# xbarin02/libdwt

Measured on AMD Instinct MI355X. Metric: Gsamples/s (= % HBM3E BW) CDF 9/7 2-D fwd float, 8192^2 5-level, higher is better.
Workload: dtype f32

## Files before the change

libdwt_amd/csrc/dwt_abi.hip:

```cpp
#include "dwt_backend.h"

#include <climits>

using namespace dwtb;

namespace {
enum OptKind { kPlain, kSweep , kBool, kNonNegative, kRing01 ,
	kUpDown01  };
struct Opt {
	const char *name;
	int *(*ref)(Ctx &);
	OptKind kind;
};
#define DWT_OPT(name_, member_, kind_) {name_, [](Ctx &c) -> int * { return &c.member_; }, kind_}
const Opt kOpts[] = {
	DWT_OPT("generic", force_generic, kSweep), DWT_OPT("eaw_two_pass", eaw_two_pass, kBool), DWT_OPT("feat_groups", feat_groups, kNonNegative), DWT_OPT("swt_fused", swt_fused, kBool), DWT_OPT("swt2d_fused", swt2d_fused, kBool), DWT_OPT("wp_fused", wp_fused, kBool), DWT_OPT("pixels_wide", pixels_wide, kBool), DWT_OPT("quant_wide", quant_wide, kBool), DWT_OPT("sparse_wide", sparse_wide, kBool), DWT_OPT("window_fused", window_fused, kNonNegative), DWT_OPT("cond_fused", cond_fused, kPlain), DWT_OPT("timefreq_tiled", tf_tiled, kBool), DWT_OPT("cpt", tune.cpt, kSweep), DWT_OPT("tile_pairs", tune.tile_pairs, kSweep),
	DWT_OPT("waves", tune.waves, kSweep), DWT_OPT("xcd_swizzle", tune.xcd_swizzle, kSweep), DWT_OPT("ring", tune.ring, kSweep),
	DWT_OPT("ring_inv", tune.ring_inv, kSweep), DWT_OPT("inv_ll_temporal", tune.inv_ll_temporal, kSweep), DWT_OPT("inv_pairs", tune.inv_pairs, kSweep), DWT_OPT("nt", tune.nt, kSweep), DWT_OPT("nt_auto", tune.nt_auto, kSweep),
	DWT_OPT("fma", fma, kSweep), DWT_OPT("fused_d", fused_d, kPlain), DWT_OPT("fuse01", fuse01, kPlain), DWT_OPT("fuse01_ring", tune.fuse01_ring, kRing01), DWT_OPT("fuse01_updown", tune.fuse01_updown, kUpDown01), DWT_OPT("ride_copy", ride_copy, kBool), DWT_OPT("ride_mib", ride_mib, kNonNegative), DWT_OPT("il_exact_borders", il_exact_borders, kPlain),
	DWT_OPT("il_inplace_shell", il_inplace_shell, kPlain), DWT_OPT("host_pipeline", host_pipeline, kPlain),
	DWT_OPT("tune_tiles", tune_tiles, kPlain), DWT_OPT("tune_in_call", tune_in_call, kBool), DWT_OPT("place_tries", place_tries, kPlain),
	DWT_OPT("place_min_mib", place_min_mib, kNonNegative), DWT_OPT("place_max_gib", place_max_gib, kNonNegative),
	DWT_OPT("vol_ip_waves", vol.ip_waves, kPlain), DWT_OPT("vol_tile_pairs", vol.tile_pairs, kPlain), DWT_OPT("vol_nt", vol.nt, kPlain),
	DWT_OPT("vol_fused", vol.fused, kPlain), DWT_OPT("vol_direct", vol.direct, kPlain), DWT_OPT("vol_whole", vol.whole, kPlain),
	DWT_OPT("vol_inplace_fused", vol.inplace_fused, kBool), DWT_OPT("vol_swizzle", vol.swizzle, kPlain), DWT_OPT("vol_rows", vol.rows, kPlain),
};
#undef DWT_OPT
const Opt *find_opt(const char *name)
{
	for (const Opt &o : kOpts)
		if (!strcmp(name, o.name))
			return &o;
	return nullptr;
}
}

#pragma GCC visibility push(default)
extern "C" {

const char *dwt_hip_last_error(void) { return g_err; }

int dwt_hip_device_count(void)
{
	int n = 0;
	if (hipGetDeviceCount(&n) != hipSuccess)
		return 0;
	return n;
}

int dwt_hip_init(void)
{
	if (g.inited)
		return 0;
	int n = 0;
	hipError_t e = hipGetDeviceCount(&n);
	if (e != hipSuccess || n <= 0)
		return fail("no HIP device available (%s); libdwt_amd has no CPU fallback", e != hipSuccess ? hipGetErrorString(e) : "0 devices");
	int dev = 0;
	const char *env = getenv("DWT_HIP_DEVICE");
	if (!env)
		env = getenv("LOCAL_RANK");
	if (g.want_device >= 0) {
		if (g.want_device >= n)
			return fail("dwt_hip_set_device(%d): the process sees %d device(s)", g.want_device, n);
		dev = g.want_device;
	} else if (env) {
		dev = atoi(env) % n;
	}
	HIP_TRY(hipSetDevice(dev));
	hipDeviceProp_t prop;
	HIP_TRY(hipGetDeviceProperties(&prop, dev));
	snprintf(g.devname, sizeof(g.devname), "%s (%s, %d CUs)", prop.name, prop.gcnArchName, prop.multiProcessorCount);
	if (!strstr(prop.gcnArchName, "gfx950"))
		return fail("device %d is %s; this library carries gfx950 code only", dev, prop.gcnArchName);
	g.device = dev;
	g.inited = true;
	return 0;
}

int dwt_hip_set_device(int device)
{
	if (device < 0)
		return fail("dwt_hip_set_device(%d): bad device index", device);
	if (g.inited && g.device != device) {
		dwt_hip_finish();
		g.inited = false;
	}
	g.want_device = device;
	return check_inited();
}

int dwt_hip_get_device(void)
{
	return g.inited ? g.device : -1;
}

void dwt_hip_finish(void)
{
	if (!g.inited)
		return;
	hipStreamSynchronize(g.stream);
	if (g.ll_external) {
		g.ll[0] = g.ll[1] = Buf{};
		g.ll_external = false;
	}
	for (Buf *b : g.bufs())
		drop(*b);
	for (hipEvent_t &e : g.dl_ev) {
		if (e)
			hipEventDestroy(e);
		e = nullptr;
	}
	for (auto &row : g.pipe_ev)
		for (hipEvent_t &e : row) {
			if (e)
				hipEventDestroy(e);
			e = nullptr;
		}
	if (g.up)
		hipStreamDestroy(g.up);
	if (g.down)
		hipStreamDestroy(g.down);
	g.up = g.down = nullptr;
	if (g.pin)
		hipHostFree(g.pin);
	g.pin = nullptr;
	g.pin_bytes = 0;
	if (g.switch_ev)
		hipEventDestroy(g.switch_ev);
	g.switch_ev = nullptr;
	for (auto &ev : g.prof_events) {
		hipEventDestroy(ev.first);
		hipEventDestroy(ev.second);
	}
	g.prof_events.clear();
	g.prof_used = 0;
	g.tile_cache.clear();
	g.place_n = 0;
	g.place_best = -1;
}

const char *dwt_hip_device_name(void)
{
	if (check_inited())
		return "";
	return g.devname;
}

void dwt_hip_set_stream(void *s)
{
	hipStream_t ns = (hipStream_t)s;
	if (g.inited && ns != g.stream) {
		hipStreamCaptureStatus a = hipStreamCaptureStatusNone, b = hipStreamCaptureStatusNone;
		const bool plain = hipStreamIsCapturing(g.stream, &a) == hipSuccess && a == hipStreamCaptureStatusNone &&
			hipStreamIsCapturing(ns, &b) == hipSuccess && b == hipStreamCaptureStatusNone;
		if (plain && (g.switch_ev || hipEventCreateWithFlags(&g.switch_ev, hipEventDisableTiming) == hipSuccess) &&
			hipEventRecord(g.switch_ev, g.stream) == hipSuccess)
			(void)hipStreamWaitEvent(ns, g.switch_ev, 0);
		(void)hipGetLastError();
	}
	g.stream = ns;
}

int dwt_hip_set_workspace(void *band0, size_t bytes0, void *band1, size_t bytes1)
{
	if (check_inited())
		return 1;
	HIP_TRY(hipStreamSynchronize(g.stream));
	if (!g.ll_external) {
		drop(g.ll[0]);
		drop(g.ll[1]);
	}
	if (!band0 || !band1) {
		g.ll[0] = g.ll[1] = Buf{};
		g.ll_external = false;
		return 0;
	}
	if (!dwt_hip_is_device_pointer(band0) || !dwt_hip_is_device_pointer(band1) || ((uintptr_t)band0 & 15) || ((uintptr_t)band1 & 15))
		return fail("dwt_hip_set_workspace takes two 16-byte aligned device buffers");
	g.ll[0] = Buf{band0, bytes0};
	g.ll[1] = Buf{band1, bytes1};
	g.ll_external = true;
	return 0;
}

int dwt_hip_fill_workspace(unsigned word)
{
	if (check_inited())
		return 1;
	for (Buf *b : g.bufs()) {
		if (!b->p || !b->bytes)
			continue;
		const size_t words = b->bytes / 4;
		if (words)
			HIP_TRY(hipMemsetD32Async((hipDeviceptr_t)b->p, (int)word, words, g.stream));
		for (size_t k = 4 * words; k < b->bytes; k++)
			HIP_TRY(hipMemsetD8Async((hipDeviceptr_t)((char *)b->p + k), (unsigned char)(word >> (8 * (k & 3))), 1, g.stream));
	}
	cond_forget_warnings();
	return 0;
}

int dwt_hip_placement_report(double *ms, int n)
{
	for (int i = 0; i < n && i < g.place_n; i++)
		ms[i] = g.place_ms[i];
	return g.place_n;
}


void dwt_hip_sync(void)
{
	if (g.inited)
		hipStreamSynchronize(g.stream);
}

int dwt_hip_set_option(const char *name, int value)
{
	const Opt *o = name ? find_opt(name) : nullptr;
	if (!o)
		return fail("unknown option '%s'", name ? name : "(null)");
	if (o->kind == kRing01 && value != 0 && !fwd01_has_ring(value))
		return fail("option fuse01_ring: 0, 8 or 16 (the fused pair has no kernel with a ring of %d rows)", value);
	if (o->kind == kUpDown01 && !fwd01_has_updown(value))
		return fail("option fuse01_updown: -1 (the rule), 0, 1 or 2, not %d", value);
	if (o->kind == kSweep || o->kind == kRing01 || o->kind == kUpDown01)
		g.tile_cache.clear();
	*o->ref(g) = o->kind == kBool ? (value ? 1 : 0) : (o->kind == kNonNegative && value < 0) ? 0 : value;
	return 0;
}

int dwt_hip_get_option(const char *name)
{
	if (!name)
		return -1;
	if (!strcmp(name, "tune_in_call"))
		return may_measure() && !g.tuning ? 1 : 0;
	if (!strcmp(name, "place_last_tries"))
		return g.place_n;
	if (!strcmp(name, "place_last_best"))
		return g.place_best;
	if (!strcmp(name, "stat_launches"))
		return (int)(g.stat_launches & 0x7fffffff);
	if (!strcmp(name, "stat_allocs"))
		return (int)(g.stat_allocs & 0x7fffffff);
	if (!strcmp(name, "tile_cache_size"))
		return (int)g.tile_cache.size();
	if (!strcmp(name, "fuse01_last_choice"))
		return g.stat_choice01;
	if (!strcmp(name, "fuse01_last_updown"))
		return g.stat_updown01;
	const Opt *o = find_opt(name);
	return o ? *o->ref(g) : -1;
}

int dwt_hip_is_device_pointer(const void *p)
{
	hipPointerAttribute_t at;
	hipError_t e = hipPointerGetAttributes(&at, p);
	if (e != hipSuccess) {
		(void)hipGetLastError();
		return 0;
	}
	return at.type == hipMemoryTypeDevice || at.type == hipMemoryTypeManaged;
}

void *dwt_hip_malloc(size_t bytes)
{
	if (check_inited())
		return nullptr;
	void *p = nullptr;
	if (hipMalloc(&p, bytes) != hipSuccess) {
		fail("hipMalloc(%zu) failed", bytes);
		return nullptr;
	}
	return p;
}

void dwt_hip_free(void *p)
{
	dev_free(p);
}

void *dwt_hip_malloc_host(size_t bytes)
{
	if (check_inited())
		return nullptr;
	void *p = nullptr;
	if (hipHostMalloc(&p, bytes, hipHostMallocDefault) != hipSuccess) {
		fail("hipHostMalloc(%zu) failed", bytes);
		return nullptr;
	}
	return p;
}

void dwt_hip_free_host(void *p)
{
	if (p)
		hipHostFree(p);
}

int dwt_hip_memcpy_h2d(void *d, const void *h, size_t n)
{
	if (check_inited())
		return 1;
	HIP_TRY(hipMemcpyAsync(d, h, n, hipMemcpyHostToDevice, g.stream));
	HIP_TRY(hipStreamSynchronize(g.stream));
	return 0;
}

int dwt_hip_memcpy_d2h(void *h, const void *d, size_t n)
{
	if (check_inited())
		return 1;
	HIP_TRY(hipMemcpyAsync(h, d, n, hipMemcpyDeviceToHost, g.stream));
	HIP_TRY(hipStreamSynchronize(g.stream));
	return 0;
}

void dwt_hip_prof_enable(int on)
{
	if (g.inited)
		prof_drain();
	g.prof_on = on;
	g.prof_ms = 0;
	g.prof_launches = 0;
}

int dwt_hip_prof_read_levels(double *ms_sum, int *launches, int n)
{
	if (prof_drain())
		return 1;
	for (int i = 0; i < n && i < 16; i++) {
		ms_sum[i] = g.prof_level_ms[i];
		launches[i] = g.prof_level_n[i];
		g.prof_level_ms[i] = 0;
		g.prof_level_n[i] = 0;
	}
	g.prof_ms = 0;
	g.prof_launches = 0;
	return 0;
}

int dwt_hip_prof_read(double *ms, int *launches)
{
	if (prof_drain())
		return 1;
	if (ms)
		*ms = g.prof_ms;
	if (launches)
		*launches = g.prof_launches;
	g.prof_ms = 0;
	g.prof_launches = 0;
	for (int i = 0; i < 16; i++) {
		g.prof_level_ms[i] = 0;
		g.prof_level_n[i] = 0;
	}
	return 0;
}
int dwt_hip_transform2d(int wavelet, int inverse, const void *src, void *dst, int stride_x, int stride_y,
	int sox, int soy, int six, int siy, int *j, int decompose_one, int zero_padding)
{
	if (check_inited())
		return 1;
	Wavelet w;
	if (!wavelet_of(wavelet, &w))
		return fail("unknown wavelet %d", wavelet);
	if (!src || !dst || !j)
		return fail("null pointer argument");
	Call2d c = call2d(w, {src, dst}, {(long)stride_x});
	const int es = c.es;
	if (sox <= 0 || soy <= 0 || six < 0 || siy < 0 || six > sox || siy > soy)
		return fail("bad sizes: outer %dx%d inner %dx%d", sox, soy, six, siy);
	const Geom ge{sox, soy, six, siy};
	const bool dev_src = dwt_hip_is_device_pointer(src), dev_dst = dwt_hip_is_device_pointer(dst);
	if (dev_src != dev_dst)
		return fail("src and dst must both be host or both be device pointers");

	if (dev_dst && stride_y == es && stride_x % es == 0 && stride_x >= sox * es && (uintptr_t)src % es == 0 && (uintptr_t)dst % es == 0) {
		Img s{(char *)src, stride_x, es}, d{(char *)dst, stride_x, es};
		if (!inverse && !decompose_one && (*j < 0 || *j >= 2) && place_ll_scratch(c, s, d, ge, *j, 1, 0, 0))
			return 1;
		return inverse ? inverse2d(c, s, d, ge, *j, decompose_one, zero_padding, 1, 0, 0)
		               : forward2d(c, s, d, ge, j, decompose_one, zero_padding, 1, 0, 0);
	}
	if (dev_dst && (stride_y < es || (long)stride_x < (long)(sox - 1) * stride_y + es))
		return fail("device image: stride_y %d must be >= %d and stride_x %d >= (width-1)*stride_y + %d", stride_y, es, stride_x, es);

	if (!dev_dst && ge.dense() && stride_y == es && es == 4) {
		const int rc = inverse ? host_inverse_pipelined(c, src, dst, stride_x, sox, soy, *j, decompose_one)
		                       : host_forward_pipelined(c, src, dst, stride_x, sox, soy, j, decompose_one);
		if (rc >= 0)
			return rc;
	}
	const bool s2 = (src != dst);
	const Frame fs{(void *)src, stride_x, stride_y, es, sox, soy, dev_dst}, fd{dst, stride_x, stride_y, es, sox, soy, dev_dst};
	Img A;
	if (frame_stage(fs, g.frame_a, &A) || grow(g.frame_b, (size_t)A.sx * soy))
		return 1;
	const long pitch = A.sx;
	const Img B{(char *)g.frame_b.p, pitch, es};
	c = call2d(w, {A.p, B.p}, {pitch});
	const int so_min = sox < soy ? sox : soy, so_max = sox > soy ? sox : soy;
	const int j_lim = ceil_log2(decompose_one ? so_max : so_min);
	const int j_eff = (*j < 0 || *j > j_lim) ? j_lim : *j;
	const bool writes_all = ge.dense() && j_eff >= 1;
	if (s2 && writes_all) {
	} else if (s2) {
		if (frame_pack(fd, B.p, pitch))
			return 1;
	} else {
		if (copy_rect(B, 0, 0, A, 0, 0, sox, soy))
			return 1;
	}
	int rc;
	if (s2 || ge.dense()) {
		rc = inverse ? inverse2d(c, A, B, ge, *j, decompose_one, zero_padding, 1, 0, 0)
		             : forward2d(c, A, B, ge, j, decompose_one, zero_padding, 1, 0, 0);
	} else {
		rc = inverse ? inverse2d(c, B, B, ge, *j, decompose_one, zero_padding, 1, 0, 0)
		             : forward2d(c, B, B, ge, j, decompose_one, zero_padding, 1, 0, 0);
	}
	if (rc)
		return rc;
	return frame_unpack(fd, B.p, pitch);
}

int dwt_hip_transform1d_batch(int wavelet, int inverse, const void *src, void *dst, size_t line_stride, int elem_stride,
	int n_lines, int size_o, int size_i, int *j, int zero_padding)
{
	if (check_inited())
		return 1;
	if (wavelet != DWT_HIP_CDF97_S && wavelet != DWT_HIP_CDF53_S && wavelet != DWT_HIP_INTERP53_S)
		return fail("1-D transforms exist for DWT_HIP_CDF97_S, DWT_HIP_CDF53_S and DWT_HIP_INTERP53_S only (wavelet %d)", wavelet);
	Wavelet w;
	wavelet_of(wavelet, &w);
	if (!src || !dst || !j)
		return fail("null pointer argument");
	if (n_lines < 0 || size_o < 0 || size_i < 0 || size_i > size_o)
		return fail("bad sizes: %d lines, outer %d inner %d", n_lines, size_o, size_i);
	if (elem_stride < 4 || line_stride > (size_t)LONG_MAX / 2)
		return fail("bad strides: line %zu bytes, element %d bytes", line_stride, elem_stride);
	return transform1d(w, inverse != 0, src, dst, (long)line_stride, elem_stride, n_lines, size_o, size_i, j, zero_padding);
}

int dwt_hip_transform1d(int wavelet, int inverse, const void *src, void *dst, int stride, int size_o, int size_i, int *j,
	int zero_padding)
{
	return dwt_hip_transform1d_batch(wavelet, inverse, src, dst, 0, stride, 1, size_o, size_i, j, zero_padding);
}

int dwt_hip_transform2d_batch(int wavelet, int inverse, const void *src, void *dst, size_t batch_stride, int batch,
	int stride_x, int size_x, int size_y, int *j)
{
	if (check_inited())
		return 1;
	Wavelet w;
	if (!wavelet_of(wavelet, &w))
		return fail("unknown wavelet %d", wavelet);
	const Call2d c = call2d(w, {src, dst}, {(long)stride_x, (long)batch_stride});
	const int es = c.es;
	if (!src || !dst || !j || batch < 1 || batch > 65535)
		return fail("bad argument (batch must be 1..65535)");
	if (!dwt_hip_is_device_pointer(src) || !dwt_hip_is_device_pointer(dst))
		return fail("batched transforms take device pointers");
	if ((stride_x % es) || stride_x < size_x * es || (batch_stride % es) || batch_stride < (size_t)stride_x * size_y)
		return fail("bad strides");
	if (batch > 1 && src == dst)
		return fail("in-place batches are not supported; use distinct src and dst");
	const Geom ge{size_x, size_y, size_x, size_y};
	Img s{(char *)src, stride_x, es}, d{(char *)dst, stride_x, es};
	if (c.line_passes_only() && batch > 1) {
		const int j_in = *j;
		for (int b = 0; b < batch; b++) {
			const Img sb{s.p + (size_t)b * batch_stride, stride_x, es}, db{d.p + (size_t)b * batch_stride, stride_x, es};
			*j = j_in;
			if (inverse ? inverse2d(c, sb, db, ge, *j, 0, 0, 1, 0, 0) : forward2d(c, sb, db, ge, j, 0, 0, 1, 0, 0))
				return 1;
		}
		return 0;
	}
	if (!inverse && (*j < 0 || *j >= 2) && place_ll_scratch(c, s, d, ge, *j, batch, (long)batch_stride, (long)batch_stride))
		return 1;
	return inverse ? inverse2d(c, s, d, ge, *j, 0, 0, batch, (long)batch_stride, (long)batch_stride)
	               : forward2d(c, s, d, ge, j, 0, 0, batch, (long)batch_stride, (long)batch_stride);
}

int dwt_hip_conv_show(int is_int, const void *src, void *dst, int stride_x, int stride_y, int size_x, int size_y)
{
	if (check_inited())
		return 1;
	if (!dwt_hip_is_device_pointer(src) || !dwt_hip_is_device_pointer(dst))
		return fail("dwt_hip_conv_show takes device images (host images: dwt_util_conv_show_s/_i)");
	if (stride_y != 4 || (stride_x & 3))
		return fail("device images need stride_y == 4 and stride_x a multiple of 4");
	hipError_t e = launch_conv_show(is_int != 0, src, dst, stride_x, size_x, size_y, g.stream);
	if (e != hipSuccess)
		return fail("conv_show launch failed: %s", hipGetErrorString(e));
	return 0;
}

int dwt_hip_compare(int is_int, const void *ptr1, const void *ptr2, int stride_x, int stride_y, int size_x, int size_y)
{
	if (check_inited())
		return -1;
	if (!dwt_hip_is_device_pointer(ptr1) || !dwt_hip_is_device_pointer(ptr2)) {
		fail("dwt_hip_compare takes device images (host images: dwt_util_compare_s/_i)");
		return -1;
	}
	if (stride_y != 4 || (stride_x & 3)) {
		fail("device images need stride_y == 4 and stride_x a multiple of 4");
		return -1;
	}
	static thread_local unsigned *counter = nullptr;
	if (!counter && hipMalloc((void **)&counter, sizeof(unsigned)) != hipSuccess) {
		fail("hipMalloc failed");
		return -1;
	}
	unsigned host = 0;
	if (hipMemsetAsync(counter, 0, sizeof(unsigned), g.stream) != hipSuccess ||
		launch_compare(is_int != 0, ptr1, ptr2, stride_x, size_x, size_y, counter, g.stream) != hipSuccess ||
		hipMemcpyAsync(&host, counter, sizeof(unsigned), hipMemcpyDeviceToHost, g.stream) != hipSuccess ||
		hipStreamSynchronize(g.stream) != hipSuccess) {
		fail("compare failed: %s", hipGetErrorString(hipGetLastError()));
		return -1;
	}
	return host ? 1 : 0;
}

}
#pragma GCC visibility pop
```

libdwt_amd/csrc/dwt_backend.h:

```cpp
#pragma once
#include "../../include/libdwt_hip.h"
#include "dwt_kernels.h"

#include <hip/hip_runtime.h>
#include <stdarg.h>
#include <stdio.h>
#include <stdlib.h>
#include <string.h>
#include <algorithm>
#include <array>
#include <condition_variable>
#include <functional>
#include <initializer_list>
#include <map>
#include <mutex>
#include <thread>
#include <unistd.h>
#include <utility>
#include <vector>

namespace dwtb {
using namespace dwt;

struct Buf {
	void *p = nullptr;
	size_t bytes = 0;
};

struct Ctx {
	bool inited = false;
	int device = 0;
	int want_device = -1;
	hipStream_t stream = nullptr;
	char devname[256] = {0};
	Buf stage_img;
	Buf ll[2];
	bool ll_external = false;
	Buf frame_a, frame_b;
	Buf vol_out;
	Buf vol_host[2];
	Buf eaw_w, eaw_ll[2];
	Buf feat_ws;
	Buf swt_ws;
	Buf cond_ws;
	Buf band_ws;
	Buf nterm_ws;
	Buf half_f32;
	Buf px_pix, px_planes, px_tmp;
	Buf wp_ws;
	Buf win_ws;
	Buf q_coef, q_index, q_planes, q_ws;
	Buf sp_planes, sp_pos, sp_val, sp_ws;
	auto bufs()
	{
		return std::array{&stage_img, &ll[0], &ll[1], &frame_a, &frame_b, &vol_out, &vol_host[0], &vol_host[1], &eaw_w, &eaw_ll[0], &eaw_ll[1], &feat_ws, &swt_ws, &cond_ws, &band_ws, &nterm_ws, &half_f32, &px_pix, &px_planes, &px_tmp, &wp_ws, &q_coef, &q_index, &q_planes, &q_ws, &win_ws, &sp_planes, &sp_pos, &sp_val, &sp_ws};
	}
	hipEvent_t dl_ev[8] = {};
	hipEvent_t switch_ev = nullptr;
	hipStream_t up = nullptr, down = nullptr;
	hipEvent_t pipe_ev[3][16] = {};
	int host_pipeline = 1;
	void *pin = nullptr;
	size_t pin_bytes = 0;
	int feat_groups = 0;
	int tf_tiled = 1;
	int cond_fused = -1;
	int swt2d_fused = 1;
	int wp_fused = 1;
	int pixels_wide = 1;
	int quant_wide = 1;
	int sparse_wide = 1;
	int window_fused = 1;
	int swt_fused = 1;
	SweepTuning tune;
	VolTuning vol;
	int force_generic = 0;
	int eaw_two_pass = 0;
	int fma = 0;
	int il_temporal = 0;
	int il_inplace_shell = 1;
	int il_exact_borders = 1;
	int tune_tiles = 1;
	std::map<unsigned long long, int> tile_cache;
	int place_tries = 4;
	int place_min_mib = 1024;
	int place_max_gib = 0;
	int tune_in_call = -1;
	bool tuning = false;
	bool placing = false;
	long stat_launches = 0, stat_allocs = 0;
	int stat_choice01 = 0;
	int stat_updown01 = 0;
	double place_ms[8] = {0};
	int place_n = 0, place_best = -1;
	int fused_d = 1;
	int fuse01 = 1;
	int ride_copy = 1;
	int ride_mib = 32;
	int prof_on = 0;
	std::vector<std::pair<hipEvent_t, hipEvent_t>> prof_events;
	std::vector<int> prof_tag;
	size_t prof_used = 0;
	double prof_ms = 0;
	int prof_launches = 0;
	double prof_level_ms[16] = {0};
	int prof_level_n[16] = {0};
};

extern thread_local Ctx g;
extern thread_local char g_err[512];
struct Call2d {
	Wavelet w;
	int es;
	bool aligned;
	bool line_passes_only() const { return es == 2 && !aligned; }
};
Call2d call2d(Wavelet w, std::initializer_list<const void *> ptrs, std::initializer_list<long> strides);
inline Wavelet sweep32_wavelet(Wavelet w) { return (g.fma && w == kCdf97S) ? kCdf97SFma : w; }

int fail(const char *fmt, ...);
int launched(hipError_t e, const char *family, const char *what);
int check_dev_align(std::initializer_list<const void *> ptrs, std::initializer_list<long> strides);
inline bool overlap(const void *a, size_t na, const void *b, size_t nb)
{
	const uintptr_t pa = (uintptr_t)a, pb = (uintptr_t)b;
	return na && nb && pa < pb + nb && pb < pa + na;
}

static_assert(facts(kInterp53S).id == DWT_HIP_INTERP53_S && facts(kCdf53I16).id == DWT_HIP_CDF53_I16 && facts(kCdf97H).id == DWT_HIP_CDF97_H, "kWaveletFacts");
static inline bool wavelet_of(int id, Wavelet *w)
{
	for (int k = 0; id >= 0 && k < kWavelets; k++)
		if (kWaveletFacts[k].id == id) {
			*w = (Wavelet)k;
			return true;
		}
	return false;
}

#define HIP_TRY(expr)                                                                          \
	do {                                                                                       \
		hipError_t e_ = (expr);                                                                \
		if (e_ != hipSuccess)                                                                  \
			return fail("%s failed: %s (%s:%d)", #expr, hipGetErrorString(e_), __FILE__, __LINE__); \
	} while (0)

inline int ceil_div_pow2(int i, int j) { return (i + (1 << j) - 1) >> j; }
inline int ceil_log2(int x)
{
	int n = 0;
	while (n < 31 && (1 << n) < x)
		n++;
	return n;
}
inline long align_up(long v, long a) { return (v + a - 1) / a * a; }

struct Img {
	char *p;
	long sx;
	int es = 4;
};

struct Geom {
	int sox, soy, six, siy;
	int Wo(int j) const { return ceil_div_pow2(sox, j); }
	int Ho(int j) const { return ceil_div_pow2(soy, j); }
	int Wi(int j) const { return ceil_div_pow2(six, j); }
	int Hi(int j) const { return ceil_div_pow2(siy, j); }
	bool dense() const { return sox == six && soy == siy; }
};

int grow(Buf &b, size_t need);
void dev_free(void *p);
void drop(Buf &b);
int grant_range(const void *p, int owner, const int *devices, int n_devices);
int copy_rect_on(hipStream_t st, Img dst, long dx, long dy, Img src, long sx_, long sy_, long w, long h);
int copy_rect(Img dst, long dx, long dy, Img src, long sx_, long sy_, long w, long h);
int zero_rect(Img img, long x, long y, long w, long h);
struct Frame {
	void *p;
	long sx, sy;
	int es, w, h;
	bool dev;
};
int frame_check(const Frame &f);
int frame_pack(const Frame &f, void *dense, long pitch);
int frame_unpack(const Frame &f, const void *dense, long pitch);
inline long frame_pitch(long es, long w) { return align_up(es * w, 256); }
int frame_stage(const Frame &f, Buf &buf, Img *dense);
int frame_pack_stack(Frame f, int n, long plane_stride, void *stack, long pitch);
int frame_unpack_stack(Frame f, int n, long plane_stride, const void *stack, long pitch);
int host_volume_xfer(bool to_device, void *dev, size_t d_sy, size_t d_sz, void *host, size_t h_sy, size_t h_sz, int nx, int ny, int nz);
int generic_pass(Wavelet w, bool inverse, bool rows, Img in, Img out, int frame_w, int frame_h, int n_lines, int N, int hoff);
size_t ll_band_bytes(const Geom &ge, int k, int batch, int es);
int timed_forward(const Call2d &c, Img s, Img d, const Geom &ge, int levels, int batch, long sb, long db, double *ms);
int place_ll_scratch(const Call2d &c, Img s, Img d, const Geom &ge, int levels, int batch, long sb, long db);
int tune2d(const Call2d &c, bool inverse, Img s, Img d, const Geom &ge, int levels, int batch, long sb, long db);
bool stream_is_capturing();
bool may_measure();
int tuned_tile_pairs(Wavelet w, const FwdLevelArgs &a);
int tuned_tile_pairs(Wavelet w, const InvLevelArgs &a);
int tuned_tile_pairs01(Wavelet w, const FwdLevelArgs &a);
int tuned_updown01(Wavelet w, const FwdLevelArgs &a, const SweepTuning &t);
enum TileUse { kTileFwd, kTileInv, kTileFwd01 };
void apply_tile_choice(int choice, SweepTuning *t, TileUse use);
int forward2d(const Call2d &c, Img src, Img dst, const Geom &ge, int *jp, int decompose_one, int zero_padding, int batch, long src_bstride, long dst_bstride);
int inverse2d(const Call2d &c, Img src, Img dst, const Geom &ge, int j_max, int decompose_one, int zero_padding, int batch, long src_bstride, long dst_bstride);
bool level_fused_ok(const Call2d &c, const Geom &ge, int j);
int transform1d(Wavelet w, bool inverse, const void *src, void *dst, long line_stride, long elem_stride, int n_lines,
	int so, int si, int *jp, int zero_padding);
int host_forward_pipelined(const Call2d &c, const void *src, void *dst, int stride_x, int W, int H, int *jp, int decompose_one);
int host_inverse_pipelined(const Call2d &c, const void *src, void *dst, int stride_x, int W, int H, int j_max, int decompose_one);
bool swt_fused_ok(const void *src, long ls, long es, int N);
int swt_device(Wavelet w, const char *src, long ls, long es, int n_lines, int N, int level0, int levels, char *dst_h, long h_es,
	char *dst_l, long l_es, int l_mode, long plane_stride, long dls, int border = kSwtReplicate);
void cond_forget_warnings();
int band_abs_median(const void *ptr, long bstride, int batch, long stride_x, int fw, int fh, int x0, int y0, int w, int h, float *med);
struct Side {
	const void *p;
	size_t extent;
	bool dense;
};
inline bool mul_add(long *acc, long count, long stride)
{
	long t;
	return !__builtin_mul_overflow(count, stride, &t) && !__builtin_add_overflow(*acc, t, acc);
}
inline bool all16(std::initializer_list<uintptr_t> v)
{
	uintptr_t o = 0;
	for (uintptr_t x : v)
		o |= x;
	return o % 16 == 0;
}
inline int nt_for(size_t out_bytes) { return out_bytes > ((size_t)128 << 20); }
int mirror(const Side &s, Buf &buf, bool upload, char **dev, bool *is_host);
int mirror_back(const Side &s, const Buf &buf);
int prof_drain();
void prof_before(int level = 0);
void prof_after(int level = 0);
int check_inited();

}
```

libdwt_amd/csrc/dwt_backend.hip:

```cpp
#include "dwt_backend.h"

namespace dwtb {

thread_local Ctx g;
thread_local char g_err[512] = "";

int fail(const char *fmt, ...)
{
	va_list ap;
	va_start(ap, fmt);
	vsnprintf(g_err, sizeof(g_err), fmt, ap);
	va_end(ap);
	return 1;
}

int launched(hipError_t e, const char *family, const char *what)
{
	g.stat_launches++;
	return e == hipSuccess ? 0 : fail("%s %s launch failed: %s", family, what, hipGetErrorString(e));
}

static bool dword_aligned(std::initializer_list<const void *> ptrs, std::initializer_list<long> strides)
{
	bool ok = true;
	for (const void *p : ptrs)
		ok = ok && (uintptr_t)p % 4 == 0;
	for (long s : strides)
		ok = ok && s % 4 == 0;
	return ok;
}

int check_dev_align(std::initializer_list<const void *> ptrs, std::initializer_list<long> strides)
{
	return dword_aligned(ptrs, strides) ? 0 : fail("device memory takes strides and addresses that are multiples of 4 bytes");
}

Call2d call2d(Wavelet w, std::initializer_list<const void *> ptrs, std::initializer_list<long> strides)
{
	return Call2d{w, elem_size(w), dword_aligned(ptrs, strides)};
}

int grow(Buf &b, size_t need)
{
	if (b.bytes >= need)
		return 0;
	if (b.p) {
		HIP_TRY(hipStreamSynchronize(g.stream));
		drop(b);
	}
	HIP_TRY(hipMalloc(&b.p, need));
	g.stat_allocs++;
	b.bytes = need;
	return 0;
}

void drop(Buf &b)
{
	if (b.p)
		dev_free(b.p);
	b = Buf{};
}

struct Rect {
	long dx, dy, sx, sy, w, h;
};
static CopyRects make_copy_rects(Img dst, Img src, const Rect *rc, int n, int policy)
{
	CopyRects r{};
	r.n = 0;
	r.policy = policy;
	for (int k = 0; k < n && r.n < 3; k++) {
		if (rc[k].w <= 0 || rc[k].h <= 0)
			continue;
		const int i = r.n++;
		r.src[i] = src.p + rc[k].sy * src.sx + rc[k].sx * src.es;
		r.dst[i] = dst.p + rc[k].dy * dst.sx + rc[k].dx * dst.es;
		r.spitch[i] = src.sx;
		r.dpitch[i] = dst.sx;
		r.wbytes[i] = (int)(rc[k].w * dst.es);
		r.h[i] = (int)rc[k].h;
	}
	return r;
}

static int copy_staged(Img dst, Img src, const Rect *rc, int n, int policy)
{
	if (dst.es != 2)
		return launched(launch_copy_rects(make_copy_rects(dst, src, rc, n, policy), g.stream), "rectangle", "copy");
	for (int k = 0; k < n; k++)
		if (copy_rect(dst, rc[k].dx, rc[k].dy, src, rc[k].sx, rc[k].sy, rc[k].w, rc[k].h))
			return 1;
	return 0;
}

struct RideCopy {
	CopyRects r;
	int next = 0, total = 0;
	bool on = false;
	int share(size_t own_bytes, int carriers_after) const
	{
		const int left = total - next;
		const int small = std::min(left, g.ride_mib * 32);
		if (carriers_after <= 0)
			return left;
		if (own_bytes <= ((size_t)32 << 20))
			return small;
		return std::max(small, left - carriers_after * g.ride_mib * 32);
	}
	int flush()
	{
		if (!on || next >= total)
			return 0;
		const int from = next;
		next = total;
		return launched(launch_copy_rects_range(r, from, total, g.stream), "rectangle", "copy");
	}
};

int copy_rect_on(hipStream_t st, Img dst, long dx, long dy, Img src, long sx_, long sy_, long w, long h)
{
	if (w <= 0 || h <= 0)
		return 0;
	HIP_TRY(hipMemcpy2DAsync(dst.p + dy * dst.sx + dx * dst.es, dst.sx, src.p + sy_ * src.sx + sx_ * src.es, src.sx, w * dst.es, h,
		hipMemcpyDeviceToDevice, st));
	return 0;
}
int copy_rect(Img dst, long dx, long dy, Img src, long sx_, long sy_, long w, long h)
{
	return copy_rect_on(g.stream, dst, dx, dy, src, sx_, sy_, w, h);
}

int zero_rect(Img img, long x, long y, long w, long h)
{
	if (w <= 0 || h <= 0)
		return 0;
	HIP_TRY(hipMemset2DAsync(img.p + y * img.sx + x * img.es, img.sx, 0, w * img.es, h, g.stream));
	return 0;
}

int generic_pass(Wavelet w, bool inverse, bool rows, Img in, Img out, int frame_w, int frame_h, int n_lines, int N, int hoff)
{
	if (n_lines <= 0 || N <= 0)
		return 0;
	if (N == 1 && facts(w).lone) {
		if (in.p != out.p)
			return copy_rect(out, 0, 0, in, 0, 0, frame_w, frame_h);
		return 0;
	}
	const bool alias = in.p == out.p;
	Img dst = out;
	if (alias) {
		if (grow(g.stage_img, (size_t)out.sx * frame_h))
			return 1;
		dst = Img{(char *)g.stage_img.p, out.sx, out.es};
		if (copy_rect(dst, 0, 0, out, 0, 0, frame_w, frame_h))
			return 1;
	} else if (in.sx != out.sx) {
		return fail("generic pass: source and destination pitches differ (%ld vs %ld)", in.sx, out.sx);
	}
	if (launched(launch_line_pass(w, inverse, in.p, dst.p, rows ? in.sx : in.es, rows ? in.es : in.sx, n_lines, N, hoff, !rows, g.stream), "line", "pass"))
		return 1;
	if (alias && copy_rect(out, 0, 0, dst, 0, 0, frame_w, frame_h))
		return 1;
	return 0;
}

void prof_before(int level)
{
	g.stat_launches++;
	if (!g.prof_on || (g.prof_on == 1 && level != 0))
		return;
	if (g.prof_tag.size() <= g.prof_used)
		g.prof_tag.resize(g.prof_used + 1);
	g.prof_tag[g.prof_used] = level;
	if (g.prof_used == g.prof_events.size()) {
		hipEvent_t a, b;
		hipEventCreate(&a);
		hipEventCreate(&b);
		g.prof_events.push_back({a, b});
	}
	hipEventRecord(g.prof_events[g.prof_used].first, g.stream);
}

void prof_after(int level)
{
	if (!g.prof_on || (g.prof_on == 1 && level != 0))
		return;
	hipEventRecord(g.prof_events[g.prof_used].second, g.stream);
	g.prof_used++;
}

int prof_drain()
{
	if (g.prof_used == 0)
		return 0;
	HIP_TRY(hipStreamSynchronize(g.stream));
	for (size_t i = 0; i < g.prof_used; i++) {
		float ms = 0;
		HIP_TRY(hipEventElapsedTime(&ms, g.prof_events[i].first, g.prof_events[i].second));
		const int lv = g.prof_tag[i] & 15;
		g.prof_level_ms[lv] += ms;
		g.prof_level_n[lv]++;
		if (lv == 0) {
			g.prof_ms += ms;
			g.prof_launches++;
		}
	}
	g.prof_used = 0;
	return 0;
}

long ll_pitch_elems(int w) { return align_up(w, 4); }
static char *ll_band(int k) { return (char *)g.ll[k].p; }

size_t ll_band_bytes(const Geom &ge, int k, int batch, int es)
{
	return (size_t)ll_pitch_elems(ge.Wo(k + 1)) * ge.Ho(k + 1) * es * batch + 64;
}

int ensure_ll(const Geom &ge, int batch, int es)
{
	for (int k = 0; k < 2; k++) {
		if (g.ll_external) {
			if (g.ll[k].bytes < ll_band_bytes(ge, k, batch, es))
				return fail("the caller's workspace (dwt_hip_set_workspace) is too small: band %d needs %zu bytes", k, ll_band_bytes(ge, k, batch, es));
			continue;
		}
		if (grow(g.ll[k], ll_band_bytes(ge, k, batch, es)))
			return 1;
	}
	return 0;
}

bool level_fused_ok(const Call2d &c, const Geom &ge, int j)
{
	return !g.force_generic && (c.es == 4 || (c.es == 2 ? c.aligned : g.fused_d != 0)) && ge.Wi(j) == ge.Wo(j) && ge.Hi(j) == ge.Ho(j) && ge.Wo(j) >= 2 &&
		ge.Ho(j) >= 2;
}
static bool pair01_ok(const Call2d &c, const Geom &ge, int J, int batch)
{
	const int W = ge.Wo(0), H = ge.Ho(0);
	if (!g.fuse01 || g.fma || J < 2 || !level_fused_ok(c, ge, 0) || !level_fused_ok(c, ge, 1) || !fwd01_can(c.w, W, H))
		return false;
	const SweepTuning &t = g.tune;
	if (t.cpt == 4 || t.ring == 8 || (t.nt & 8) || (t.tile_pairs & 1))
		return false;
	if (g.fuse01 >= 2)
		return true;
	const long ntx = fwd01_tiles(W), nty = ((H >> 1) + 63) / 64;
	return ntx * nty * batch >= 32768;
}

static int half_level_begin(Img cur, Img dst, int Wo, int Ho, Img *fcur, Img *fdst)
{
	const long fp = align_up((long)Wo * 4, 256);
	if (grow(g.half_f32, (size_t)fp * Ho * 2))
		return 1;
	*fcur = Img{(char *)g.half_f32.p, fp, 4};
	if (launched(launch_half_frame_cvt(true, cur.p, cur.sx, fcur->p, fp, Wo, Ho, g.stream), "binary16 frame", "widening"))
		return 1;
	*fdst = *fcur;
	if (cur.p != dst.p) {
		*fdst = Img{(char *)g.half_f32.p + (size_t)fp * Ho, fp, 4};
		if (launched(launch_half_frame_cvt(true, dst.p, dst.sx, fdst->p, fp, Wo, Ho, g.stream), "binary16 frame", "widening"))
			return 1;
	}
	return 0;
}

static int half_level_end(Img fdst, Img dst, int Wo, int Ho)
{
	return launched(launch_half_frame_cvt(false, dst.p, dst.sx, fdst.p, fdst.sx, Wo, Ho, g.stream), "binary16 frame", "narrowing");
}

static int generic_level(const Call2d &c, bool inverse, Img in, Img out, int Wo, int Ho, int Wi, int Hi, int Wh, int Hh)
{
	const WaveletFacts &f = facts(c.w);
	const bool cols_first = inverse ? f.cols_inv : f.cols_fwd;
	Img lc = in, ld = out;
	if (widened(c.w) && half_level_begin(in, out, Wo, Ho, &lc, &ld))
		return 1;
	const bool dense = Wi == Wo && Hi == Ho && Wo >= 2 && Ho >= 2;
	if (dense && grow(g.stage_img, (size_t)ld.sx * Ho))
		return 1;
	for (int pass = 0; pass < 2; pass++) {
		const bool rows = cols_first != (pass == 0);
		if (f.skip1 && (rows ? Wo : Ho) <= 1)
			continue;
		const Img to = dense && pass == 0 ? Img{(char *)g.stage_img.p, ld.sx, ld.es} : ld;
		if (generic_pass(f.line_as, inverse, rows, lc, to, Wo, Ho, rows ? Ho : Wo, rows ? Wi : Hi, rows ? Wh : Hh))
			return 1;
		lc = to;
	}
	return widened(c.w) ? half_level_end(ld, out, Wo, Ho) : 0;
}

static hipError_t sweep_fwd(const Call2d &c, const FwdLevelArgs &a, const SweepTuning &t, hipStream_t s)
{
	return c.es == 8 ? launch_fwd_level_d(c.w, a, t, s)
	     : c.es == 4 ? launch_fwd_level(sweep32_wavelet(c.w), a, t, s)
	     : widened(c.w) ? launch_fwd_level_h(c.w, a, t, s)
	                    : launch_fwd_level_i16(c.w, a, t, s);
}

static hipError_t sweep_inv(const Call2d &c, const InvLevelArgs &a, const SweepTuning &t, hipStream_t s)
{
	return c.es == 8 ? launch_inv_level_d(c.w, a, t, s)
	     : c.es == 4 ? launch_inv_level(sweep32_wavelet(c.w), a, t, s)
	     : widened(c.w) ? launch_inv_level_h(c.w, a, t, s)
	                    : launch_inv_level_i16(c.w, a, t, s);
}

int forward2d(const Call2d &c, Img src, Img dst, const Geom &ge, int *jp, int decompose_one, int zero_padding,
	int batch, long src_bstride, long dst_bstride)
{
	const int so_min = ge.sox < ge.soy ? ge.sox : ge.soy, so_max = ge.sox > ge.soy ? ge.sox : ge.soy;
	const int j_limit = ceil_log2(decompose_one ? so_max : so_min);
	if (*jp < 0 || *jp > j_limit)
		*jp = j_limit;
	const int J = *jp;
	if (J == 0)
		return 0;
	const Wavelet w = c.w;
	const int es = c.es;
	if (ensure_ll(ge, batch, es))
		return 1;

	int ll_in = -1;
	Img cur = src;
	RideCopy ride;
	auto carriers_from = [&](int j0) {
		int n = 0;
		for (int j = j0; j < J && level_fused_ok(c, ge, j); j++)
			n += es == 4 && sweep_ride_ok(g.tune, ge.Wo(j), ge.Ho(j), batch, false);
		return n;
	};
	for (int j = 0; j < J; j++) {
		const int Wo = ge.Wo(j), Ho = ge.Ho(j), Wi = ge.Wi(j), Hi = ge.Hi(j);
		const int Wd = ge.Wo(j + 1), Hd = ge.Ho(j + 1);
		if (level_fused_ok(c, ge, j)) {
			const bool pair = j == 0 && ll_in < 0 && cur.p != dst.p && pair01_ok(c, ge, J, batch);
			const int jl = pair ? j + 1 : j;
			const bool last = (jl == J - 1) || !level_fused_ok(c, ge, jl + 1);
			FwdLevelArgs a;
			a.W = Wo;
			a.H = Ho;
			a.batch = batch;
			bool detour = false;
			if (ll_in < 0) {
				a.in = cur.p;
				a.in_pitch = cur.sx / es;
				a.in_bstride = (cur.p == src.p ? src_bstride : dst_bstride) / es;
				detour = (cur.p == dst.p);
			} else {
				a.in = ll_band(ll_in);
				a.in_pitch = ll_pitch_elems(Wo);
				a.in_bstride = a.in_pitch * Ho;
			}
			Img hdst = dst;
			long h_bstride = dst_bstride;
			if (detour) {
				if (batch != 1)
					return fail("in-place batches are not supported; use distinct src and dst");
				if (grow(g.stage_img, (size_t)dst.sx * Ho))
					return 1;
				hdst = Img{(char *)g.stage_img.p, dst.sx, es};
				h_bstride = 0;
				a.temporal = (g.ride_copy && carriers_from(j + 1) > 0) ? 0 : 1;
			}
			a.out_h = hdst.p;
			a.h_pitch = hdst.sx / es;
			a.h_bstride = h_bstride / es;
			const int ll_out = last ? -1 : (ll_in < 0 ? (jl & 1) : 1 - ll_in);
			if (last) {
				a.out_ll = hdst.p;
				a.ll_pitch = a.h_pitch;
				a.ll_bstride = a.h_bstride;
			} else {
				a.out_ll = ll_band(ll_out);
				a.ll_pitch = ll_pitch_elems(ge.Wo(jl + 1));
				a.ll_bstride = a.ll_pitch * ge.Ho(jl + 1);
			}
			SweepTuning tune = g.tune;
			if (pair)
				g.stat_choice01 = 0;
			if (es == 4 && tune.tile_pairs <= 0) {
				const int choice = pair ? tuned_tile_pairs01(w, a) : tuned_tile_pairs(w, a);
				apply_tile_choice(choice, &tune, pair ? kTileFwd01 : kTileFwd);
				if (pair)
					g.stat_choice01 = choice;
			}
			if (pair) {
				const int dir = tuned_updown01(w, a, tune);
				if (dir >= 0)
					tune.fuse01_updown = dir;
				g.stat_updown01 = fwd01_updown(tune, a.W, a.H, a.batch);
			}
			if (ride.on && ride.next < ride.total && es == 4 && sweep_ride_ok(tune, Wo, Ho, batch, false)) {
				a.ride = &ride.r;
				a.ride_lo = ride.next;
				a.ride_hi = ride.next + ride.share((size_t)Wo * Ho * es, carriers_from(j + 1));
				ride.next = a.ride_hi;
			}
			prof_before(j);
			hipError_t e = pair ? launch_fwd01(a, tune, g.stream) : sweep_fwd(c, a, tune, g.stream);
			prof_after(j);
			if (e != hipSuccess)
				return fail("forward level %d launch failed: %s", j, hipGetErrorString(e));
			if (detour) {
				const Rect rc[3] = {{Wd, 0, Wd, 0, Wo - Wd, Ho}, {0, Hd, 0, Hd, Wd, Ho - Hd}, {0, 0, 0, 0, last ? Wd : 0, Hd}};
				if (es == 4) {
					ride.r = make_copy_rects(dst, hdst, rc, 3, 3);
					ride.total = copy_rects_plan(&ride.r);
					ride.next = 0;
					ride.on = g.ride_copy && ride.total > 0 && carriers_from(j + 1) > 0;
				}
				if (!ride.on && copy_staged(dst, hdst, rc, 3, 3))
					return 1;
			}
			ll_in = ll_out;
			cur = dst;
			j = jl;
			continue;
		}

		if (ride.flush())
			return 1;
		if (batch != 1)
			return fail("batched transforms need dense frames with both sides >= 2 at every level");
		if (ll_in >= 0) {
			Img s{ll_band(ll_in), ll_pitch_elems(Wo) * es, es};
			if (copy_rect(dst, 0, 0, s, 0, 0, Wo, Ho))
				return 1;
			ll_in = -1;
			cur = dst;
		}
		if (generic_level(c, false, cur, dst, Wo, Ho, Wi, Hi, Wd, Hd))
			return 1;
		cur = dst;
		if (zero_padding) {
			const int nl_x = (Wi + 1) >> 1, nh_x = Wi >> 1, nl_y = (Hi + 1) >> 1, nh_y = Hi >> 1;
			if (zero_rect(dst, nl_x, 0, Wd - nl_x, Ho) || zero_rect(dst, Wd + nh_x, 0, (Wo - Wd) - nh_x, Ho) ||
				zero_rect(dst, 0, nl_y, Wo, Hd - nl_y) || zero_rect(dst, 0, Hd + nh_y, Wo, (Ho - Hd) - nh_y))
				return 1;
		}
	}
	return ride.flush();
}

int inverse2d(const Call2d &c, Img src, Img dst, const Geom &ge, int j_max, int decompose_one, int zero_padding,
	int batch, long src_bstride, long dst_bstride)
{
	const int so_min = ge.sox < ge.soy ? ge.sox : ge.soy, so_max = ge.sox > ge.soy ? ge.sox : ge.soy;
	int J = ceil_log2(decompose_one ? so_max : so_min);
	if (j_max >= 0 && j_max < J)
		J = j_max;
	if (J == 0) {
		if (src.p != dst.p && copy_rect(dst, 0, 0, src, 0, 0, ge.six, ge.siy))
			return 1;
		return 0;
	}
	const Wavelet w = c.w;
	const int es = c.es;
	if (ensure_ll(ge, batch, es))
		return 1;

	auto fused_ok = [&](int j) { return level_fused_ok(c, ge, j - 1); };

	Img cur = src;
	long cur_bstride = src_bstride;
	int ll_in = -1;
	bool copied = false;
	RideCopy ride;
	if (src.p == dst.p && batch == 1 && J >= 2 && g.ride_copy && es == 4) {
		bool all = true;
		int carriers = 0;
		for (int j = J; j >= 1; j--)
			all = all && fused_ok(j);
		for (int j = J; j >= 2; j--)
			carriers += sweep_ride_ok(g.tune, ge.Wo(j - 1), ge.Ho(j - 1), batch, true);
		if (all && carriers > 0) {
			const int Ws = ge.Wo(1), Hs = ge.Ho(1), Wo = ge.Wo(0), Ho = ge.Ho(0);
			if (grow(g.stage_img, (size_t)dst.sx * Ho))
				return 1;
			Img st{(char *)g.stage_img.p, dst.sx, es};
			const Rect rc[2] = {{Ws, 0, Ws, 0, Wo - Ws, Ho}, {0, Hs, 0, Hs, Ws, Ho - Hs}};
			ride.r = make_copy_rects(st, src, rc, 2,  0);
			ride.total = copy_rects_plan(&ride.r);
			ride.on = ride.total > 0;
		}
	}
	for (int j = J; j >= 1; j--) {
		const int Ws = ge.Wo(j), Hs = ge.Ho(j);
		const int Wo = ge.Wo(j - 1), Ho = ge.Ho(j - 1);
		const int Wi = ge.Wi(j - 1), Hi = ge.Hi(j - 1);
		if (fused_ok(j)) {
			InvLevelArgs a;
			a.W = Wo;
			a.H = Ho;
			a.batch = batch;
			a.in_h = cur.p;
			a.h_pitch = cur.sx / es;
			a.h_bstride = cur_bstride / es;
			if (ll_in < 0) {
				a.in_ll = cur.p;
				a.ll_pitch = cur.sx / es;
				a.ll_bstride = cur_bstride / es;
			} else {
				a.in_ll = ll_band(ll_in);
				a.ll_pitch = ll_pitch_elems(Ws);
				a.ll_bstride = a.ll_pitch * Hs;
			}
			const bool last = (j == 1);
			int ll_out = -1;
			if (last) {
				a.out = dst.p;
				a.out_pitch = dst.sx / es;
				a.out_bstride = dst_bstride / es;
				if (cur.p == dst.p) {
					if (batch != 1)
						return fail("in-place batches are not supported; use distinct src and dst");
					if (grow(g.stage_img, (size_t)dst.sx * Ho))
						return 1;
					Img st{(char *)g.stage_img.p, dst.sx, es};
					const Rect rc[3] = {{Ws, 0, Ws, 0, Wo - Ws, Ho}, {0, Hs, 0, Hs, Ws, Ho - Hs}, {0, 0, 0, 0, ll_in < 0 ? Ws : 0, Hs}};
					if (ride.on) {
						if (ride.flush())
							return 1;
					} else if (copy_staged(st, cur, rc, 3,  0))
						return 1;
					a.in_h = st.p;
					a.h_bstride = 0;
					if (ll_in < 0)
						a.in_ll = st.p;
				}
			} else {
				ll_out = j & 1;
				a.out = ll_band(ll_out);
				a.out_pitch = ll_pitch_elems(Wo);
				a.out_bstride = a.out_pitch * Ho;
				a.temporal_out = g.tune.inv_ll_temporal && src.p != dst.p && (size_t)Wo * Ho * es * batch <= ((size_t)128 << 20);
			}
			SweepTuning tune = g.tune;
			if (tune.inv_pairs <= 0)
				tune.inv_pairs = src.p == dst.p ? 32 : 16;
			if (es == 4 && tune.tile_pairs <= 0)
				apply_tile_choice(tuned_tile_pairs(w, a), &tune, kTileInv);
			if (ride.on && !last && ride.next < ride.total && sweep_ride_ok(tune, Wo, Ho, batch, true)) {
				int after = 0;
				for (int m = j - 1; m >= 2; m--)
					after += sweep_ride_ok(g.tune, ge.Wo(m - 1), ge.Ho(m - 1), batch, true);
				a.ride = &ride.r;
				a.ride_lo = ride.next;
				a.ride_hi = ride.next + ride.share((size_t)Wo * Ho * es, after);
				ride.next = a.ride_hi;
			}
			prof_before(j - 1);
			hipError_t e = sweep_inv(c, a, tune, g.stream);
			prof_after(j - 1);
			if (e != hipSuccess)
				return fail("inverse level %d launch failed: %s", j, hipGetErrorString(e));
			ll_in = ll_out;
			continue;
		}

		if (batch != 1)
			return fail("batched transforms need dense frames with both sides >= 2 at every level");
		if (src.p != dst.p && !copied) {
			if (copy_rect(dst, 0, 0, src, 0, 0, ge.six, ge.siy))
				return 1;
			copied = true;
		}
		cur = dst;
		cur_bstride = dst_bstride;
		if (ll_in >= 0) {
			Img s{ll_band(ll_in), ll_pitch_elems(Ws) * es, es};
			if (copy_rect(dst, 0, 0, s, 0, 0, Ws, Hs))
				return 1;
			ll_in = -1;
		}
		if (generic_level(c, true, dst, dst, Wo, Ho, Wi, Hi, Ws, Hs))
			return 1;
		if (zero_padding) {
			if (zero_rect(dst, Wi, 0, Wo - Wi, Ho) || zero_rect(dst, 0, Hi, Wo, Ho - Hi))
				return 1;
		}
	}
	return 0;
}

int check_inited()
{
	if (!g.inited && dwt_hip_init())
		return 1;
	return 0;
}

}
```

Measured before the change: 651.9.

## Fuse deeper forward level pairs into the two-level kernel

Generalises the fused level-0/1 forward kernel so that later even levels (j>=2) can also run as a two-level pair reading from the LL ping-pong buffers. This is gated on the level-0 pair having been chosen by size, and on a minimum tile count at the deeper level. Deep pairs get default ring, up/down and tile_pairs settings when tuning gives none. The aim is to save a launch and one intermediate LL round trip through memory per pair. The risk is that the fused kernel runs with low occupancy on small deep levels.

```diff
diff --git a/libdwt_amd/csrc/dwt_abi.hip b/libdwt_amd/csrc/dwt_abi.hip
--- a/libdwt_amd/csrc/dwt_abi.hip
+++ b/libdwt_amd/csrc/dwt_abi.hip
@@ -17,7 +17,7 @@
 	DWT_OPT("generic", force_generic, kSweep), DWT_OPT("eaw_two_pass", eaw_two_pass, kBool), DWT_OPT("feat_groups", feat_groups, kNonNegative), DWT_OPT("swt_fused", swt_fused, kBool), DWT_OPT("swt2d_fused", swt2d_fused, kBool), DWT_OPT("wp_fused", wp_fused, kBool), DWT_OPT("pixels_wide", pixels_wide, kBool), DWT_OPT("quant_wide", quant_wide, kBool), DWT_OPT("sparse_wide", sparse_wide, kBool), DWT_OPT("window_fused", window_fused, kNonNegative), DWT_OPT("cond_fused", cond_fused, kPlain), DWT_OPT("timefreq_tiled", tf_tiled, kBool), DWT_OPT("cpt", tune.cpt, kSweep), DWT_OPT("tile_pairs", tune.tile_pairs, kSweep),
 	DWT_OPT("waves", tune.waves, kSweep), DWT_OPT("xcd_swizzle", tune.xcd_swizzle, kSweep), DWT_OPT("ring", tune.ring, kSweep),
 	DWT_OPT("ring_inv", tune.ring_inv, kSweep), DWT_OPT("inv_ll_temporal", tune.inv_ll_temporal, kSweep), DWT_OPT("inv_pairs", tune.inv_pairs, kSweep), DWT_OPT("nt", tune.nt, kSweep), DWT_OPT("nt_auto", tune.nt_auto, kSweep),
-	DWT_OPT("fma", fma, kSweep), DWT_OPT("fused_d", fused_d, kPlain), DWT_OPT("fuse01", fuse01, kPlain), DWT_OPT("fuse01_ring", tune.fuse01_ring, kRing01), DWT_OPT("fuse01_updown", tune.fuse01_updown, kUpDown01), DWT_OPT("ride_copy", ride_copy, kBool), DWT_OPT("ride_mib", ride_mib, kNonNegative), DWT_OPT("il_exact_borders", il_exact_borders, kPlain),
+	DWT_OPT("fma", fma, kSweep), DWT_OPT("fused_d", fused_d, kPlain), DWT_OPT("fuse01", fuse01, kPlain), DWT_OPT("fuse_deep", fuse_deep, kNonNegative), DWT_OPT("fuse01_ring", tune.fuse01_ring, kRing01), DWT_OPT("fuse01_updown", tune.fuse01_updown, kUpDown01), DWT_OPT("ride_copy", ride_copy, kBool), DWT_OPT("ride_mib", ride_mib, kNonNegative), DWT_OPT("il_exact_borders", il_exact_borders, kPlain),
 	DWT_OPT("il_inplace_shell", il_inplace_shell, kPlain), DWT_OPT("host_pipeline", host_pipeline, kPlain),
 	DWT_OPT("tune_tiles", tune_tiles, kPlain), DWT_OPT("tune_in_call", tune_in_call, kBool), DWT_OPT("place_tries", place_tries, kPlain),
 	DWT_OPT("place_min_mib", place_min_mib, kNonNegative), DWT_OPT("place_max_gib", place_max_gib, kNonNegative),
@@ -250,6 +250,8 @@
 		return g.stat_choice01;
 	if (!strcmp(name, "fuse01_last_updown"))
 		return g.stat_updown01;
+	if (!strcmp(name, "fuse_deep_last"))
+		return g.stat_deep_pairs;
 	const Opt *o = find_opt(name);
 	return o ? *o->ref(g) : -1;
 }
diff --git a/libdwt_amd/csrc/dwt_backend.h b/libdwt_amd/csrc/dwt_backend.h
--- a/libdwt_amd/csrc/dwt_backend.h
+++ b/libdwt_amd/csrc/dwt_backend.h
@@ -95,6 +95,8 @@
 	int place_n = 0, place_best = -1;
 	int fused_d = 1;
 	int fuse01 = 1;
+	int fuse_deep = 1;
+	int stat_deep_pairs = 0;
 	int ride_copy = 1;
 	int ride_mib = 32;
 	int prof_on = 0;
diff --git a/libdwt_amd/csrc/dwt_backend.hip b/libdwt_amd/csrc/dwt_backend.hip
--- a/libdwt_amd/csrc/dwt_backend.hip
+++ b/libdwt_amd/csrc/dwt_backend.hip
@@ -237,18 +237,32 @@
 	return !g.force_generic && (c.es == 4 || (c.es == 2 ? c.aligned : g.fused_d != 0)) && ge.Wi(j) == ge.Wo(j) && ge.Hi(j) == ge.Ho(j) && ge.Wo(j) >= 2 &&
 		ge.Ho(j) >= 2;
 }
-static bool pair01_ok(const Call2d &c, const Geom &ge, int J, int batch)
-{
-	const int W = ge.Wo(0), H = ge.Ho(0);
-	if (!g.fuse01 || g.fma || J < 2 || !level_fused_ok(c, ge, 0) || !level_fused_ok(c, ge, 1) || !fwd01_can(c.w, W, H))
+static long pair_tiles(const Geom &ge, int j, int batch)
+{
+	return (long)fwd01_tiles(ge.Wo(j)) * (((ge.Ho(j) >> 1) + 63) / 64) * batch;
+}
+
+static bool pair_legal(const Call2d &c, const Geom &ge, int J, int j)
+{
+	if ((j & 1) || g.fma || j + 1 >= J || !level_fused_ok(c, ge, j) || !level_fused_ok(c, ge, j + 1) || !fwd01_can(c.w, ge.Wo(j), ge.Ho(j)))
 		return false;
 	const SweepTuning &t = g.tune;
-	if (t.cpt == 4 || t.ring == 8 || (t.nt & 8) || (t.tile_pairs & 1))
+	return !(t.cpt == 4 || t.ring == 8 || (t.nt & 8) || (t.tile_pairs & 1));
+}
+
+static bool pair01_ok(const Call2d &c, const Geom &ge, int J, int batch, bool *by_size)
+{
+	*by_size = g.fuse01 && pair_legal(c, ge, J, 0) && pair_tiles(ge, 0, batch) >= 32768;
+	return *by_size || (g.fuse01 >= 2 && pair_legal(c, ge, J, 0));
+}
+
+constexpr long kDeepTiles = 2048;
+constexpr int kDeepRing = 8, kDeepUpDown = 1, kDeepPairs = 128;
+static bool pair_deep_ok(const Call2d &c, const Geom &ge, int J, int batch, int j, bool pair01_by_size)
+{
+	if (!g.fuse_deep || j < 2 || !pair_legal(c, ge, J, j))
 		return false;
-	if (g.fuse01 >= 2)
-		return true;
-	const long ntx = fwd01_tiles(W), nty = ((H >> 1) + 63) / 64;
-	return ntx * nty * batch >= 32768;
+	return g.fuse_deep >= 2 || (pair01_by_size && pair_tiles(ge, j, batch) >= kDeepTiles);
 }
 
 static int half_level_begin(Img cur, Img dst, int Wo, int Ho, Img *fcur, Img *fdst)
@@ -329,6 +343,8 @@
 	int ll_in = -1;
 	Img cur = src;
 	RideCopy ride;
+	bool pair01_by_size = false;
+	g.stat_deep_pairs = 0;
 	auto carriers_from = [&](int j0) {
 		int n = 0;
 		for (int j = j0; j < J && level_fused_ok(c, ge, j); j++)
@@ -339,7 +355,13 @@
 		const int Wo = ge.Wo(j), Ho = ge.Ho(j), Wi = ge.Wi(j), Hi = ge.Hi(j);
 		const int Wd = ge.Wo(j + 1), Hd = ge.Ho(j + 1);
 		if (level_fused_ok(c, ge, j)) {
-			const bool pair = j == 0 && ll_in < 0 && cur.p != dst.p && pair01_ok(c, ge, J, batch);
+			bool by_size = false;
+			const bool pair = j == 0 ? ll_in < 0 && cur.p != dst.p && pair01_ok(c, ge, J, batch, &by_size)
+			                         : ll_in >= 0 && !(ride.on && ride.next < ride.total) && pair_deep_ok(c, ge, J, batch, j, pair01_by_size);
+			if (j == 0)
+				pair01_by_size = pair && by_size;
+			else if (pair)
+				g.stat_deep_pairs++;
 			const int jl = pair ? j + 1 : j;
 			const bool last = (jl == J - 1) || !level_fused_ok(c, ge, jl + 1);
 			FwdLevelArgs a;
@@ -382,19 +404,27 @@
 				a.ll_bstride = a.ll_pitch * ge.Ho(jl + 1);
 			}
 			SweepTuning tune = g.tune;
-			if (pair)
+			if (pair && j == 0)
 				g.stat_choice01 = 0;
+			const bool deep_rule = pair && j > 0 && pair_tiles(ge, j, batch) >= kDeepTiles;
+			if (deep_rule && !tune.fuse01_ring)
+				tune.fuse01_ring = kDeepRing;
 			if (es == 4 && tune.tile_pairs <= 0) {
 				const int choice = pair ? tuned_tile_pairs01(w, a) : tuned_tile_pairs(w, a);
 				apply_tile_choice(choice, &tune, pair ? kTileFwd01 : kTileFwd);
-				if (pair)
+				if (pair && j == 0)
 					g.stat_choice01 = choice;
+				if (deep_rule && choice <= 0 && (Ho >> 1) >= 2 * kDeepPairs)
+					tune.tile_pairs = kDeepPairs;
 			}
 			if (pair) {
 				const int dir = tuned_updown01(w, a, tune);
 				if (dir >= 0)
 					tune.fuse01_updown = dir;
-				g.stat_updown01 = fwd01_updown(tune, a.W, a.H, a.batch);
+				else if (deep_rule && tune.fuse01_updown < 0)
+					tune.fuse01_updown = kDeepUpDown;
+				if (j == 0)
+					g.stat_updown01 = fwd01_updown(tune, a.W, a.H, a.batch);
 			}
 			if (ride.on && ride.next < ride.total && es == 4 && sweep_ride_ok(tune, Wo, Ho, batch, false)) {
 				a.ride = &ride.r;
```

Result: faster. 666.7, median of 6 (+2.3%).
